# xuangu-fang/Gaussian-Process-Slover-for-High-Freq-PDE

Hardware: AMD Instinct MI355X
Metric: log-joint iters/sec + fp64 Cholesky GFLOP/s, 2D Poisson 256^2, 1-8 GPU (higher is better)
Workload: dtype f64; 1 GPU; C4: 2D Poisson 256x256 Kronecker grid, Matern52_Cos_1d, Q=30, fp64; Q=30, kernel=Matern52_Cos_1d, equation=poisson_2d-sin_sin, parallelism=replicas x1 (one independent problem per GPU)

## Files before the change

gaussian-process-slover-for-high-freq-pde_amd/csrc/gpk_create.cpp:

```cpp
#include <atomic>

#include "gpk_host.h"

static std::atomic<int> g_chain_cap{0};

bool build_classes(const double* x, int n, int P, std::vector<double>& dist, std::vector<int>& cid,
                   std::vector<int>& cbase, int& vmax) {
  cid.assign((size_t)P * P, -1);
  cbase.assign((size_t)n + 1, 0);
  dist.clear();
  vmax = 0;
  double vals[CLS_VMAX];
  for (int k = 0; k < n; ++k) {
    int nv = 0;
    cbase[k] = (int)dist.size();
    for (int j = 0; j + k < n; ++j) {
      const double d = std::fabs(x[j + k] - x[j]);
      int v = 0;
      while (v < nv && !(vals[v] == d)) ++v;
      if (v == nv) {
        if (nv == CLS_VMAX) return false;
        vals[nv++] = d;
        dist.push_back(d);
      }
// ... 137 lines not shown
  A_(h->grad, L.nparams);
  A_(h->m, L.nparams);
  A_(h->v, L.nparams);
  A_(h->Up, nup);
  A_(h->kc, 2);
  A_(h->sc, 1);
  A_(h->count, 1);
  A_(h->loss_slot, 1);
  A_(h->status, 1);
  A_(h->stat_x, 2);
  A_(h->losses, LOSS_CAP);
  A_(h->diag, 8);
  for (int a = 0; a < L.naxes; ++a) {
    const int P = axis_p(L, a);
    A_(h->K[a], (size_t)P * P);
    A_(h->Kb[a], (size_t)P * P);
    A_(h->D[a], (size_t)P * P);
    A_(h->piv[a], spd_big_piv_doubles(P));
    A_(h->ldet[a], P / 32);
    A_(h->Kc[a], (size_t)P * P);
    A_(h->pst[a], 2);
    A_(h->aflag[a], 4 + P / 32);
    if (h->bigspd) A_(h->Zp[a], (size_t)3 * 128 * P);
    if (h->bigspd && h->bigwide && !(p->flags & GPK_FLAG_ONE_SWEEP_UPDATE)) {
      const int T2 = (int)((P + 127) / 128);
      std::vector<unsigned> tab;
      wide_schedule(T2, true, tab);
      A_(h->wsched[a], tab.size());
      if (hipMemcpyAsync(h->wsched[a], tab.data(), tab.size() * sizeof(unsigned), hipMemcpyHostToDevice, h->s) != hipSuccess ||
          hipStreamSynchronize(h->s) != hipSuccess)
        return fail(GPK_EHIP, "upload the update schedule");
    }
    A_(h->cflags[a], (size_t)(P / 32) * (P / 32 + (P1 + P2) / 32) + 2 * (P / 32) + 1);
    A_(h->cgran[a], (size_t)(P / 32) * 2048);
    if (hipMemsetD32Async(h->cgran[a], CHAIN_SENTINEL32, (size_t)(P / 32) * 4096, h->s) != hipSuccess)
      return fail(GPK_EHIP, "initialise the pivot-chain input slots");
    if (h->chain) {
      A_(h->PB2[a], 2 * chain_half(P, h->chain_multi));
      A_(h->cepoch[a], 4);
      if (hipMemsetD32Async(h->PB2[a], CHAIN_SENTINEL32, 4 * chain_half(P, h->chain_multi), h->s) != hipSuccess)
        return fail(GPK_EHIP, "initialise the panel slots");
    }
    if (h->chain_aug) {
      A_(h->PD[a], (size_t)P * P);
      A_(h->PBa[a], (size_t)P * (P1 + P2));
    }
    h->nldet[a] = P / 32;
  }
  if (L.dim == 2) {
    A_(h->A, nup); A_(h->Bt, nup); A_(h->S, nup); A_(h->R, nup);
    A_(h->T1, nup); A_(h->T2, nup); A_(h->X1, nup); A_(h->X2, nup);
    A_(h->W1, nup); A_(h->W2, nup); A_(h->Y1, nup); A_(h->Y2, nup);
    for (int a = 0; a < 2; ++a) {
      const int P = axis_p(L, a);
      A_(h->GK[a], (size_t)P * P);
      A_(h->GD[a], (size_t)P * P);
    }
    h->nquad = h->negap = (P1 / 16) * (P2 / 16);
  } else {
    A_(h->alpha, P1); A_(h->R, P1); A_(h->tvec, P1); A_(h->beta, P1); A_(h->rvec, P1);
    if (p->uoff) A_(h->uoff, P1);
    h->nquad = h->negap = gemv_blocks(P1);
  }
  if (shard) {
    const size_t npg = (size_t)L.naxes * 3 * QMAX;
    A_(h->sred, 2 + npg + (size_t)h->negap + (size_t)h->nquad);
    h->stat_x = h->sred;
    h->pg = h->sred + 2;
// ... 259 lines not shown
```

gaussian-process-slover-for-high-freq-pde_amd/csrc/gpk_internal.h:

```cpp
#pragma once
#include <vector>
#include <hip/hip_runtime.h>
#include <stdint.h>

namespace gpk {

constexpr int QMAX = 64;
constexpr int PADM = 32;
constexpr int NB = 32;
constexpr double SQRT5 = 2.23606797749978969641;
constexpr double TWO_PI = 6.28318530717958647692;

enum Kind { SE_COS = 0, MATERN52_COS = 1, SE = 2, MATERN52 = 3 };

__host__ __device__ inline bool kind_matern(int k) { return k == MATERN52_COS || k == MATERN52; }
__host__ __device__ inline bool kind_cos(int k) { return k == SE_COS || k == MATERN52_COS; }
inline int pad_up(int n) { return (n + PADM - 1) / PADM * PADM; }

struct AxisConst {
  double w[QMAX];
  double a[QMAX];
  double om[QMAX];
  double oml[QMAX];
};
// ... 138 lines not shown
  double* Y;
  int p;
  int n;
  double* piv;
  double* ldet;
  double* pst;
  int* status;
  unsigned int* flag;
  int wide;
  int no_quarters;
  int qfirst;
  double* Z;
  const unsigned* sched;
};
int wide_sched_stride(int T2);
void wide_schedule(int T2, bool paired, std::vector<unsigned>& tab);
hipError_t launch_spd_inverse(SpdArgs* args, int nmat, double** final_out, hipStream_t s,
                              bool pivot0_done = false);
hipError_t launch_spd_stage(SpdArgs* args, int nmat, int stage, hipStream_t s);

constexpr int CHAIN_MAX_BLOCKS = 512;
struct ChainArgs {
  double* X; double* PB; double* piv; double* ldet; double* pst; int* status;
  unsigned int* flags;
  int p, n;
  const int* cid; const double* kval; const double* dval; const double* x; double jitter;
  double* Kc; double* D;
  int tu, td;
  const double* Bu; int ldbu, bu_t;
  double* Ou; int ldou, ou_t;
  double* Od; int ldod;
  double* PBa; int ldpba;
  double* gran;
  double* PB2; unsigned int* epoch;
};
__host__ __device__ inline size_t multi_half(int p) { return (size_t)p * p + (size_t)32 * p; }
__host__ __device__ inline size_t chain_half(int p, bool multi) { return multi ? multi_half(p) : (size_t)32 * p; }
constexpr unsigned long long CHAIN_SENTINEL = 0x7ff4dead7ff4deadull;
constexpr unsigned int CHAIN_SENTINEL32 = 0x7ff4deadu;
int spd_chain_blocks(const int* p, int nmat, bool aug);
int spd_chain_capacity(int deriv, bool gather);
__host__ __device__ inline int chain_role(int m, int x, int T, int TC) {
  const int nt = T * TC, nc = 2 * (T - 1);
  auto crit = [TC](int i) { return (i & 1) ? ((i >> 1) + 1) * (TC + 1) : (i >> 1) * (TC + 1) + 1; };
  int r;
  if (m == 0) {
    if (x == nt) return nt;
    if (x >= nt - nc) return crit(x - (nt - nc));
    r = x;
  } else {
    if (x == 0) return nt;
    if (x <= nc) return crit(x - 1);
    r = x - 1 - nc;
  }
  int tile = r;
  for (int i = 0; i < nc; ++i)
    if (crit(i) <= tile) ++tile;
  return tile;
}
int spd_chain_multi_blocks(const int* p, int nmat);
int spd_chain_multi_capacity(int deriv, bool gather);
hipError_t launch_spd_chain_multi(const ChainArgs* a, int nmat, int deriv, hipStream_t s,
                                  const PrepArgs* prep = nullptr, int q = 0);
hipError_t launch_spd_chain(const ChainArgs* a, int nmat, int deriv, hipStream_t s,
                            const PrepArgs* prep = nullptr, int q = 0);

// ... 103 lines not shown
```

gaussian-process-slover-for-high-freq-pde_amd/csrc/gpk_step.cpp:

```cpp
#include <sched.h>

#include <atomic>

#include "gpk_host.h"

namespace {
const char* kStageNames1D[] = {"prep", "assemble", "spd_inverse", "gemv_alpha", "gemv_alpha_res",
                               "gemv_alpha_fix", "gemv_resid", "gemv_DtR", "gemv_beta",
                               "gemv_beta_res", "gemv_beta_fix", "pgrad_tail"};
const char* kStageNames2D[] = {"prep", "assemble", "spd_inverse", "gemm_A", "gemm_A_res",
                               "gemm_A_fix", "gemm_B", "gemm_B_res", "gemm_B_fix", "gemm_C",
                               "gemm_D", "gemm_D_res", "gemm_D_fix", "gemm_E", "pgrad_tail"};
}

static void mark(gpk_handle* h, int stage) {
  if (h->profiling) (void)hipEventRecord(h->ev[stage + 1], h->s);
}

PrepArgs make_prep(gpk_handle* h, int apply) {
  const Layout& L = h->L;
  PrepArgs P{};
  P.params = h->params;
  P.off_kp[0] = L.off_kp[0];
  P.off_kp[1] = L.off_kp[1];
// ... 19 lines not shown
  return !h->shard && h->chain && h->cls[0].ncls > 0 && h->nce_flag &&
         !(h->prob.flags & GPK_FLAG_NO_CLASS_PIPE);
}

void fill_spd(gpk_handle* h, SpdArgs* sa) {
  const Layout& L = h->L;
  for (int a = 0; a < L.naxes; ++a) {
    sa[a] = SpdArgs{};
    sa[a].X = h->K[a];
    sa[a].Y = h->Kb[a];
    sa[a].p = axis_p(L, a);
    sa[a].n = axis_n(L, a);
    sa[a].piv = h->piv[a];
    sa[a].ldet = h->ldet[a];
    sa[a].status = h->status;
    sa[a].pst = h->pst[a];
    sa[a].flag = h->aflag[a];
    sa[a].wide = h->bigwide ? 1 : 0;
    sa[a].no_quarters = (h->prob.flags & GPK_FLAG_NO_QUARTER_TILES) ? 1 : 0;
    sa[a].qfirst = (h->prob.flags & GPK_FLAG_NO_QUARTER_FIRST) ? 0 : 1;
    sa[a].Z = h->Zp[a];
    sa[a].sched = h->wsched[a];
  }
}

hipError_t launch_chain(gpk_handle* h, bool gather, double** fin, bool aug, const PrepArgs* prep) {
  const Layout& L = h->L;
  ChainArgs ca[2] = {};
  for (int a = 0; a < L.naxes; ++a) {
    ChainArgs& c = ca[a];
    c.X = h->K[a]; c.PB = h->Kb[a]; c.piv = h->piv[a]; c.ldet = h->ldet[a]; c.pst = h->pst[a];
    c.status = h->status; c.flags = h->cflags[a]; c.gran = h->cgran[a];
    c.PB2 = h->PB2[a]; c.epoch = h->cepoch[a];
    c.p = axis_p(L, a);
    c.n = axis_n(L, a);
    if (gather) {
      c.cid = h->cls[a].cid; c.kval = h->cls[a].kval; c.dval = h->cls[a].dval;
      c.x = axis_x(h, a); c.jitter = h->prob.jitter; c.Kc = h->Kc[a];
    }
    c.D = h->D[a];
    if (gather && h->cls_gemv) c.Kc = c.D = nullptr;
    if (h->chain_aug && aug) {
      c.tu = axis_p(L, 1 - a) / 32; c.td = c.p / 32;
      c.Bu = h->Up; c.ldbu = L.p2; c.bu_t = a;
      c.Ou = a ? h->Bt : h->A; c.ldou = L.p2; c.ou_t = a;
      c.Od = h->PD[a]; c.ldod = c.p;
      c.PBa = h->PBa[a]; c.ldpba = L.p1 + L.p2;
    }
    fin[a] = h->K[a];
  }
  if (h->chain_multi) return launch_spd_chain_multi(ca, L.naxes, step_deriv(h), h->s, prep, L.q);
  return launch_spd_chain(ca, L.naxes, step_deriv(h), h->s, prep, L.q);
}

hipError_t launch_inverse(gpk_handle* h, SpdArgs* sa, double** fin, bool pivot0_done) {
  if (h->bigspd) return launch_spd_inverse_big(sa, h->L.naxes, fin, h->s);
  if (h->chain) return launch_chain(h, false, fin, false);
  return launch_spd_inverse(sa, h->L.naxes, fin, h->s, pivot0_done);
}

void fill_assemble(const gpk_handle* h, AssembleArgs* aa) {
  for (int a = 0; a < h->L.naxes; ++a) {
    aa[a] = AssembleArgs{};
    aa[a].x = axis_x(h, a);
    aa[a].n = axis_n(h->L, a);
    aa[a].p = axis_p(h->L, a);
// ... 474 lines not shown
  h->fold_report = nullptr;
  if (rc != GPK_OK) return rc;
  if (pending_begin) return fail(GPK_EINVAL, "internal: the batch begin was not folded into a step");
  if (pending_report || h->shard) return check_launch(launch_step_report(*r, h->s), "step_report");
  return GPK_OK;
}

static int capture_whole(gpk_handle* h, hipGraphExec_t* slot, bool fast, int reps) {
  if (*slot) return GPK_OK;
  const StepBegin b = make_begin(h, fast);
  const StepReport rep = make_report(h, fast, reps);
  return capture_graph(h->s, slot, [&] {
    int rc = begin_batch(h, &b);
    if (rc == GPK_OK) rc = enqueue_steps(h, 1, !fast, reps, &rep);
    return end_batch(h, &rep, rc);
  });
}

static int capture_call(gpk_handle* h, bool fast) {
  return capture_whole(h, &h->g_call[fast ? 0 : 1], fast, 1);
}

static int capture_calln(gpk_handle* h, int reps) {
  const int rc = capture_whole(h, &h->g_calln[reps], true, reps);
  if (rc != GPK_OK) h->g_calln.erase(reps);
  return rc;
}

int reset_handoffs(gpk_handle* h) {
  const Layout& L = h->L;
  for (int a = 0; a < L.naxes; ++a) {
    const size_t P = axis_p(L, a), T = P / 32;
    const size_t nflags = T * (T + (L.p1 + L.p2) / 32) + 2 * T + 1;
    HIPCHK(hipMemsetD32Async(h->cgran[a], CHAIN_SENTINEL32, T * 4096, h->s));
    if (h->PB2[a]) HIPCHK(hipMemsetD32Async(h->PB2[a], CHAIN_SENTINEL32, 4 * chain_half((int)P, h->chain_multi), h->s));
    if (h->cepoch[a]) HIPCHK(hipMemsetAsync(h->cepoch[a], 0, 4 * sizeof(unsigned int), h->s));
    HIPCHK(hipMemsetAsync(h->cflags[a], 0, nflags * sizeof(unsigned int), h->s));
    HIPCHK(hipMemsetAsync(h->aflag[a], 0, (4 + P / 32) * sizeof(unsigned int), h->s));
  }
  HIPCHK(hipMemsetAsync(h->nce_flag, 0, sizeof(unsigned int), h->s));
  HIPCHK(hipStreamSynchronize(h->s));
  return GPK_OK;
}

int status_error(int st, int* status, hipStream_t s, gpk_handle* h, bool undo_batch, bool handoffs) {
  const bool timeout = handoffs && (st & 2);
  HIPCHK(hipMemsetAsync(status, 0, sizeof(int), s));
  if (timeout) TRY(reset_handoffs(h));
  if (undo_batch) {
    TRY(restore_snapshot(h));
    HIPCHK(hipStreamSynchronize(s));
  }
  const std::string msg =
      timeout ? "SPD inverse: a pivot-chain hand-off timed out (device status 2)"
              : "covariance factor is not positive definite (non-positive pivot in SPD inverse)";
  return fail(GPK_ENOTPD, undo_batch ? msg + "; the batch was undone" : msg);
}

int read_status(gpk_handle* h) {
  int st = 0;
  HIPCHK(hipMemcpyAsync(&st, h->status, sizeof(int), hipMemcpyDeviceToHost, h->s));
  HIPCHK(hipStreamSynchronize(h->s));
  return st ? status_error(st, h->status, h->s, h, false, true) : GPK_OK;
}

constexpr double FAST_GRAPH_MARGIN = 2.0;
static int read_report(gpk_handle* h, bool fast, bool* violated);
// ... 228 lines not shown
```

gaussian-process-slover-for-high-freq-pde_amd/csrc/gpk_trace.h:

```cpp
#pragma once
#include <hip/hip_runtime.h>
#include <stdint.h>

namespace gpk {

constexpr int TRACE_SLOTS = 256;
enum TraceSlot {
  SLOT_CLASS_EVAL = 0, SLOT_GATHER = 1, SLOT_PIVOT0_WAIT = 2, SLOT_PIVOT0 = 3,
  SLOT_SWEEP = 4,
  SLOT_SWEEP_PIVOT = 20,
  SLOT_PREFETCH_MISS = 36,
  SLOT_PG_GARR = 37,
  SLOT_PG_ULAST = 38,
  SLOT_CLASS_SUM = 40, SLOT_PGRAD = 41, SLOT_PG_CONTRACT = 42, SLOT_PG_GROUP = 43,
  SLOT_PG_TOP = 44, SLOT_PG_UPLANE = 45, SLOT_PG_FINAL = 46,
  SLOT_PG_START = 47, SLOT_PG_STAGED = 48, SLOT_CSUM_START = 49, SLOT_CEVAL_START = 50,
  SLOT_GATHER_START = 51, SLOT_CSUM_LOADED = 52, SLOT_CHAIN_END = 53, SLOT_CHAIN_M1 = 54,
  SLOT_LAST_FLAG = 58, SLOT_LAST_LDS = 59, SLOT_LAST_MMA = 60, SLOT_LAST_OUT = 61, SLOT_LAST_AUG = 62,
  SLOT_GEMM = 64,
  SLOT_MC_PANEL = 128,
  SLOT_MC_PIV = 144,
  SLOT_MC_LDS = 160,
  SLOT_MC_V = 176,
  SLOT_MC_PUB = 192,
  SLOT_MC_DONE = 208,
  SLOT_MC_PROD = 224,
  SLOT_MCP_IN = 64, SLOT_MCP_OUT = 240,
  SLOT_MCP_WHO_IN = 80, SLOT_MCP_WHO_OUT = 96, SLOT_MCP_MPOS = 112,
  SLOT_BIG_START = 240, SLOT_BIG_PIVTILE = 241, SLOT_BIG_PIVOT = 242, SLOT_BIG_PANEL_WAIT = 243,
  SLOT_BIG_PANEL = 244, SLOT_BIG_ROUND0 = 245, SLOT_BIG_ROUND1 = 246, SLOT_BIG_QUARTER = 247,
  SLOT_BIG_R0START = 248,
};
constexpr int BIG_PROBE_SWEEP = 8;

#ifdef GPK_TRACE
#define GPK_TRACE_TU(tu)                                                                  \
  namespace {                                                                             \
  __device__ unsigned long long trace_lo[TRACE_SLOTS], trace_hi[TRACE_SLOTS];             \
  }                                                                                       \
  void trace_fetch_##tu(uint64_t* lo, uint64_t* hi) {                                     \
    (void)hipMemcpyFromSymbol(lo, HIP_SYMBOL(trace_lo), sizeof(trace_lo));                \
    (void)hipMemcpyFromSymbol(hi, HIP_SYMBOL(trace_hi), sizeof(trace_hi));                \
  }                                                                                       \
  void trace_reset_##tu() {                                                               \
    unsigned long long lo[TRACE_SLOTS], hi[TRACE_SLOTS];                                  \
    for (int i = 0; i < TRACE_SLOTS; ++i) lo[i] = ~0ull, hi[i] = 0ull;                    \
// ... 36 lines not shown
```

gaussian-process-slover-for-high-freq-pde_amd/csrc/spdinv.hip:

```cpp
#include <algorithm>

#include "gpk_internal.h"
#include "spd_pivot.h"
#include "gpk_trace.h"
#include "prep_dev.h"

namespace gpk {

GPK_WAIT_LIMIT_SETTER(wait_limit_spdinv)

GPK_TRACE_TU(spdinv)

typedef double d4 __attribute__((ext_vector_type(4)));

constexpr int SA = 34;
constexpr int SB = 48;
struct SpdBatch {
  double* X[2];
  double* Y[2];
  int p[2];
  int T[2];
  double* piv[2];
  double* ldet[2];
  double* pst[2];
// ... 115 lines not shown
    __syncthreads();
    if (t == 0) {
      double mx = 0.0;
      for (int j = 0; j < 32; ++j) mx = fmax(mx, pv[j]);
      atomicMax(reinterpret_cast<unsigned long long*>(b.pst[m] + 1),
                (unsigned long long)__double_as_longlong(mx));
    }
    if (trb) TR_HI(SLOT_SWEEP + k);
    return;
  }
  if (!nextpiv) {
    if (trb) TR_HI(SLOT_SWEEP + k);
    return;
  }
  __syncthreads();
  if (trb) TR_LO(SLOT_SWEEP_PIVOT + k);
  const double ls = pivot_chol_inv_1w(sP, sM, pv, t, b.status[m]);
  double* piv = b.piv[m] + (size_t)(k + 1) * 1024;
  for (int e = t; e < 1024; e += 256) piv[e] = sM[(e >> 5) * SP + (e & 31)];
  if (t == 0) b.ldet[m][k + 1] = ls;
  if (trb) TR_HI(SLOT_SWEEP_PIVOT + k);
  if (trb) TR_HI(SLOT_SWEEP + k);
}

struct ChainFactor {
  double* X;
  double* PB;
  double* piv;
  double* ldet;
  double* pst;
  int* status;
  unsigned int* flags;
  double* gran;
  double* PB2;
  unsigned int* epoch;
  int piv_off;
  int p, n, T;
  const int* cid; const double* kval; const double* dval; const double* x; double jitter;
  double* Kc; double* D;
  int tu, td;
  const double* Bu; int ldbu, bu_t;
  double* Ou; int ldou, ou_t;
  double* Od; int ldod;
  double* PBa; int ldpba;
};
struct ChainBatch {
  ChainFactor f[2];
  int nmat;
  PrepArgs prep;
  int q;
  int mpos;
};

__device__ __forceinline__ void st_sc1(double* p, double v) {
  __hip_atomic_store(p, v, __ATOMIC_RELAXED, __HIP_MEMORY_SCOPE_AGENT);
}
__device__ __forceinline__ double ld_sc1(const double* p) {
  return __hip_atomic_load(const_cast<double*>(p), __ATOMIC_RELAXED, __HIP_MEMORY_SCOPE_AGENT);
}
__device__ __forceinline__ void wait_flag(unsigned int* f, int* status) {
  (void)spin_until_ge<1>(f, 1u, status);
}
__device__ __forceinline__ void signal_flag(unsigned int* f) {
  asm volatile("s_waitcnt vmcnt(0)" ::: "memory");
  __syncthreads();
  if (threadIdx.x == 0) __hip_atomic_store(f, 1u, __ATOMIC_RELAXED, __HIP_MEMORY_SCOPE_AGENT);
}

__device__ __forceinline__ double* gran_at(const ChainFactor& F, int slot, int which, int e) {
  return F.gran + (size_t)(2 * slot + which) * 1024 + e;
}
__device__ __forceinline__ bool gran_ok(double v) {
  return __double_as_longlong(v) != (long long)CHAIN_SENTINEL;
}

template <bool ONEWAVE>
__device__ __forceinline__ void chain_master(const ChainFactor& F, int T, d4 acc, double* sXJ,
                                             double* sP, double* sM, double* pv, bool trm,
                                             bool early_flag, double* lw = nullptr) {
  const int t = threadIdx.x, lane = t & 63, wv = t >> 6;
  const int wr = wv >> 1, wc = wv & 1;
  const int tx = t & 31, ty = t >> 5;
  unsigned int* piv_rdy = F.flags + F.piv_off;
  __shared__ int s_pflag;
  __builtin_amdgcn_s_setprio(3);
  auto ex = [&](int r) { return (ty + 8 * r) * 32 + tx; };
  auto ed = [&](int r) { return (16 * wr + (lane >> 4) + 4 * r) * 32 + 16 * wc + (lane & 15); };
  double gx[4], gd[4];
  auto issue = [&](int k) {
#pragma unroll
    for (int r = 0; r < 4; ++r) {
      gx[r] = ld_sc1(gran_at(F, k, 0, ex(r)));
      gd[r] = ld_sc1(gran_at(F, k, 1, ed(r)));
    }
  };
  struct PivotPrefetch {
    __device__ constexpr bool waves() const { return true; }
    decltype(issue)* f;
    int k, T;
    __device__ void early() {}
    __device__ void pre() {}
    __device__ void post() {
      if (k + 1 < T) (*f)(k);
    }
  };
  auto factor = [&](int kp) {
    if (trm && kp > 0 && kp < 17) TR_HI(SLOT_SWEEP + kp - 1);
    store_quad(sP, SP, wr, wc, lane, acc);
    __syncthreads();
    if (trm && kp > 0 && kp < 17) TR_LO(SLOT_SWEEP_PIVOT + kp - 1);
    if (trm && kp == 0) TR_LO(SLOT_PIVOT0);
    PivotPrefetch hook{&issue, kp, T};
// ... 57 lines not shown
  }
}

template <int DERIV, bool GATHER>
__global__ __launch_bounds__(256, 2) void chain_kernel(ChainBatch b) {
  const int m = blockIdx.y;
  if (m == b.nmat) {
    if (blockIdx.x == 0) publish_prep(b.prep, b.q);
    copy_snapshot(b.prep, blockIdx.x, gridDim.x);
    return;
  }
  const ChainFactor& F = b.f[m];
  const int T = F.T, p = F.p;
  const int TC = T + F.tu + F.td;
  if ((int)blockIdx.x > T * TC) return;
  const int tile = chain_role(m, (int)blockIdx.x, T, TC);
  const bool master = tile == T * TC;
  const int I = master ? 0 : tile / TC, J = master ? 0 : tile % TC;
  const bool aug = J >= T;
  const int ja = J - T;
  const int t = threadIdx.x, lane = t & 63, wv = t >> 6;
  const int wr = wv >> 1, wc = wv & 1;
  const int tx = t & 31, ty = t >> 5;
  unsigned int* panel_rdy = F.flags;
  unsigned int* piv_rdy = F.flags + T * TC;
  unsigned int* done = F.flags + T * TC + 2 * T;
  auto panel_ptr = [&](int k, int row, int col) -> double* {
    return J < T ? F.PB + (size_t)(k * 32 + row) * p + J * 32 + col
                 : F.PBa + (size_t)(k * 32 + row) * F.ldpba + ja * 32 + col;
  };
  __shared__ double sL[32 * SA];
  __shared__ double sXI[32 * SB], sXJ[32 * SB];
  __shared__ double sP[32 * SP], sM[32 * SP], pv[32];
  __shared__ unsigned int s_last;
  const unsigned ep = F.PB2 ? __hip_atomic_load(F.epoch, __ATOMIC_RELAXED, __HIP_MEMORY_SCOPE_AGENT) : 0u;
  double* PLc = F.PB2 ? F.PB2 + (size_t)(ep & 1u) * chain_half(p, false) : nullptr;

  d4 acc;
#pragma unroll
  for (int r = 0; r < 4; ++r) {
    const int i = I * 32 + 16 * wr + (lane >> 4) + 4 * r, j = J * 32 + 16 * wc + (lane & 15);
    const size_t o = (size_t)i * p + j;
    if (aug) {
      const int jl = ja * 32 + 16 * wc + (lane & 15);
      if (ja < F.tu) {
        acc[r] = F.bu_t ? F.Bu[(size_t)(jl) * F.ldbu + i] : F.Bu[(size_t)i * F.ldbu + jl];
      } else {
        const int jd = jl - 32 * F.tu;
        const size_t od = (size_t)jd * p + i;
        if (GATHER) {
          const int u = F.cid[od];
          double dv = u >= 0 ? F.dval[u] : 0.0;
          if (DERIV == 1 && u >= 0 && !(F.x[jd] - F.x[i] >= 0.0)) dv = -dv;
          acc[r] = dv;
        } else {
          acc[r] = F.D[od];
        }
      }
      continue;
    }
    if (GATHER) {
      const int u = F.cid[o];
      double kv, dv;
      if (u >= 0) {
        kv = F.kval[u];
        if (i == j) kv += F.jitter;
        dv = F.dval[u];
        if (DERIV == 1 && !(F.x[i] - F.x[j] >= 0.0)) dv = -dv;
      } else {
        kv = (i == j) ? 1.0 : 0.0;
        dv = 0.0;
      }
      if (!master) {
        if (F.Kc) F.Kc[o] = kv;
        if (DERIV && F.D) F.D[o] = dv;
      }
      acc[r] = kv;
    } else {
      acc[r] = F.X[o];
    }
  }
  auto publish_tile = [&](void) {
#pragma unroll
    for (int r = 0; r < 4; ++r) st_sc1(panel_ptr(I, 16 * wr + (lane >> 4) + 4 * r, 16 * wc + (lane & 15)), acc[r]);
    signal_flag(panel_rdy + I * TC + J);
  };
  auto chain_inputs = [&](int kk) {
    const int which = (I == kk && J == kk + 1) ? 0 : (I == J && I == kk + 1) ? 1 : -1;
    if (which < 0 || kk + 1 >= T) return;
#pragma unroll
    for (int r = 0; r < 4; ++r)
      st_sc1(gran_at(F, kk, which, (16 * wr + (lane >> 4) + 4 * r) * 32 + 16 * wc + (lane & 15)), acc[r]);
  };
  const bool trm = t == 0 && m == 0;
  if (master) {
    chain_master<true>(F, T, acc, sXJ, sP, sM, pv, trm, false, PLc);
  } else {
    if (trm && tile == 0) TR_LO(SLOT_GATHER);
    chain_inputs(0);
    if (I == 0 && J != 0) publish_tile();
    if (PLc) {
      double* PLo = F.PB2 + (size_t)((ep & 1u) ^ 1u) * chain_half(p, false);
      const int share = (T * 1024 + T * TC - 1) / (T * TC);
      const int e1 = min(T * 1024, (tile + 1) * share);
      for (int e = tile * share + t; e < e1; e += 256) PLo[e] = __longlong_as_double((long long)CHAIN_SENTINEL);
    }
  }

  for (int k = 0; k < T && !master; ++k) {
    const bool needI = I != k, needJ = J != k && J != I;
    if (I == k + 1 || (I == k + 2 && J == k + 2)) __builtin_amdgcn_s_setprio(2);
    else __builtin_amdgcn_s_setprio(0);
    if (t == 0) {
      if (needI) wait_flag(panel_rdy + k * TC + I, F.status);
      if (needJ) wait_flag(panel_rdy + k * TC + J, F.status);
    }
    __syncthreads();
    double xi[4], xj[4];
#pragma unroll
    for (int r = 0; r < 4; ++r) {
      const int row = ty + 8 * r;
      xi[r] = needI ? ld_sc1(F.PB + (size_t)(k * 32 + row) * p + I * 32 + tx) : 0.0;
      xj[r] = needJ ? ld_sc1(panel_ptr(k, row, tx)) : 0.0;
    }
    const bool trl = t == 0 && m == 0 && k == T - 1 && I == T - 1 && J == T - 1;
    double lv[4];
    if (PLc) {
      const double* Lw = PLc + (size_t)k * 1024;
      if (t == 0) {
// ... 521 lines not shown

int spd_chain_multi_blocks(const int* p, int nmat) {
  int w = 0;
  for (int m = 0; m < nmat; ++m) w = std::max(w, multi_workgroups(p[m] / 32));
  return w * nmat;
}

int spd_chain_blocks(const int* p, int nmat, bool aug) {
  int blocks = 0, cols = 0;
  for (int m = 0; m < nmat; ++m) cols += p[m] / 32;
  for (int m = 0; m < nmat; ++m) blocks += (p[m] / 32) * (p[m] / 32 + (aug ? cols : 0)) + 1;
  return blocks;
}

hipError_t launch_spd_chain(const ChainArgs* a, int nmat, int deriv, hipStream_t s,
                            const PrepArgs* prep, int q) {
  ChainBatch b{};
  b.nmat = nmat;
  if (prep) {
    b.prep = *prep;
    b.q = q;
  }
  int Tmax = 0;
  bool gather = a[0].cid != nullptr;
  for (int m = 0; m < nmat; ++m) {
    ChainFactor& f = b.f[m];
    f.X = a[m].X; f.PB = a[m].PB; f.piv = a[m].piv; f.ldet = a[m].ldet; f.pst = a[m].pst;
    f.status = a[m].status; f.flags = a[m].flags; f.p = a[m].p; f.n = a[m].n; f.T = a[m].p / 32;
    f.cid = a[m].cid; f.kval = a[m].kval; f.dval = a[m].dval; f.x = a[m].x; f.jitter = a[m].jitter;
    f.Kc = a[m].Kc; f.D = a[m].D;
    f.tu = a[m].tu; f.td = a[m].td; f.Bu = a[m].Bu; f.ldbu = a[m].ldbu; f.bu_t = a[m].bu_t;
    f.Ou = a[m].Ou; f.ldou = a[m].ldou; f.ou_t = a[m].ou_t; f.Od = a[m].Od; f.ldod = a[m].ldod;
    f.PBa = a[m].PBa; f.ldpba = a[m].ldpba;
    f.gran = a[m].gran; f.piv_off = f.T * (f.T + f.tu + f.td);
    f.PB2 = a[m].PB2; f.epoch = a[m].epoch;
    if ((a[m].cid != nullptr) != gather || !f.gran || !f.PB2 != !f.epoch) return hipErrorInvalidValue;
    Tmax = std::max(Tmax, f.T * (f.T + f.tu + f.td) + 1);
  }
  dim3 grid(Tmax, nmat + (prep ? 1 : 0));
  if (!gather)
    hipLaunchKernelGGL((chain_kernel<0, false>), grid, dim3(256), 0, s, b);
  else if (deriv == 1)
    hipLaunchKernelGGL((chain_kernel<1, true>), grid, dim3(256), 0, s, b);
  else
    hipLaunchKernelGGL((chain_kernel<2, true>), grid, dim3(256), 0, s, b);
  return hipGetLastError();
}

hipError_t launch_spd_chain_multi(const ChainArgs* a, int nmat, int deriv, hipStream_t s,
                                  const PrepArgs* prep, int q) {
  ChainBatch b{};
  b.nmat = nmat;
  if (prep) {
    b.prep = *prep;
    b.q = q;
  }
  int wmax = 0;
  const bool gather = a[0].cid != nullptr;
  for (int m = 0; m < nmat; ++m) {
    ChainFactor& f = b.f[m];
    f.X = a[m].X; f.PB = a[m].PB; f.piv = a[m].piv; f.ldet = a[m].ldet; f.pst = a[m].pst;
    f.status = a[m].status; f.flags = a[m].flags; f.p = a[m].p; f.n = a[m].n; f.T = a[m].p / 32;
    f.cid = a[m].cid; f.kval = a[m].kval; f.dval = a[m].dval; f.x = a[m].x; f.jitter = a[m].jitter;
    f.Kc = a[m].Kc; f.D = a[m].D;
    f.gran = a[m].gran; f.piv_off = f.T * f.T; f.PB2 = a[m].PB2; f.epoch = a[m].epoch;
    if ((a[m].cid != nullptr) != gather || a[m].tu || a[m].td || !f.gran || !f.PB2 || !f.epoch)
      return hipErrorInvalidValue;
// ... 59 lines not shown
```

gaussian-process-slover-for-high-freq-pde_amd/gpk/_lib.py:

```python
import ctypes
import os

import numpy as np

_HERE = os.path.dirname(os.path.abspath(__file__))
LIB_PATH = os.environ.get("GPK_LIB_PATH") or os.path.join(_HERE, "_lib", "libgpk.so")

GPK_OK, GPK_EINVAL, GPK_ENOTPD, GPK_EHIP, GPK_ERCCL, GPK_ENOMEM, GPK_ENODEV = range(7)
GPK_FLAG_FORCE_BIG_GEMM = 1
GPK_FLAG_FORCE_BIG_SPD = 2
GPK_FLAG_FORCE_SMALL_SPD = 4
GPK_FLAG_FORCE_HUGE_GEMM = 8
GPK_FLAG_NO_FAST_GRAPH = 16
GPK_FLAG_FAST_FIRST = 32
GPK_FLAG_NO_DCLASS = 64
GPK_FLAG_NO_CHAIN = 128
GPK_FLAG_NO_CHAIN_AUG = 256
GPK_FLAG_FORCE_WIDE_SPD = 512
GPK_FLAG_FORCE_NARROW_SPD = 1024
GPK_FLAG_SPLIT_FACTORS = 2048
GPK_FLAG_FORCE_CHAIN_MULTI = 4096
GPK_FLAG_REFINE_ALL = 8192
GPK_FLAG_NO_REFINE = 16384
GPK_FLAG_MATRIX_GEMV = 32768
GPK_FLAG_NO_QUARTER_TILES = 65536
GPK_FLAG_DD_CONTRACTION = 131072
GPK_FLAG_NO_DD_CONTRACTION = 262144
GPK_FLAG_ONE_SWEEP_UPDATE = 524288
GPK_FLAG_NO_QUARTER_FIRST = 1048576
GPK_FLAG_REFINE_FWD1_ONLY = 2097152
GPK_FLAG_NO_CLASS_BINS = 4194304
GPK_FLAG_NO_CLASS_PIPE = 8388608
GPK_INV_SWEEP, GPK_INV_CHAIN, GPK_INV_CHAIN_AUG, GPK_INV_BIG, GPK_INV_BIG_WIDE, GPK_INV_CHAIN_MULTI = range(6)
INV_PATH_NAMES = {0: "sweep", 1: "chain", 2: "chain_aug", 3: "big", 4: "big_wide", 5: "chain_multi"}
KIND_IDS = {"SE_Cos_1d": 0, "Matern52_Cos_1d": 1, "SE_1d": 2, "Matern52_1d": 3}
EQ_IDS = {"poisson": 0, "allencahn": 1, "advection": 2}

_dp = ctypes.POINTER(ctypes.c_double)
_ip = ctypes.POINTER(ctypes.c_int32)


class GPKError(RuntimeError):
    def __init__(self, code, msg):
        super().__init__(f"libgpk error {code}: {msg}")
        self.code = code


class NotPositiveDefinite(GPKError):
    pass


class gpk_problem(ctypes.Structure):
    _fields_ = [
        ("dim", ctypes.c_int32), ("eq", ctypes.c_int32), ("kind", ctypes.c_int32),
        ("n1", ctypes.c_int32), ("n2", ctypes.c_int32), ("q", ctypes.c_int32),
        ("x1", _dp), ("x2", _dp), ("src", _dp), ("bvals", _dp), ("bidx", _ip),
        ("nb", ctypes.c_int32),
        ("jitter", ctypes.c_double), ("llk_weight", ctypes.c_double),
        ("logdet", ctypes.c_double), ("beta", ctypes.c_double),
        ("lr", ctypes.c_double), ("b1", ctypes.c_double), ("b2", ctypes.c_double),
        ("eps", ctypes.c_double),
        ("device", ctypes.c_int32), ("flags", ctypes.c_int32),
        ("uoff", _dp),
    ]

# ... 135 lines not shown
```

include/gpk.h:

```cpp
#ifndef GPK_H_
#define GPK_H_

#include <stdint.h>

#ifdef __cplusplus
extern "C" {
#endif

#define GPK_ABI_VERSION 2

enum {
  GPK_OK = 0,
  GPK_EINVAL = 1,
  GPK_ENOTPD = 2,
  GPK_EHIP = 3,
  GPK_ERCCL = 4,
  GPK_ENOMEM = 5,
  GPK_ENODEV = 6
};

enum { GPK_SE_COS = 0, GPK_MATERN52_COS = 1, GPK_SE = 2, GPK_MATERN52 = 3 };

enum { GPK_POISSON = 0, GPK_ALLENCAHN = 1, GPK_ADVECTION = 2 };

// ... 13 lines not shown
  double llk_weight;
  double logdet;
  double beta;
  double lr, b1, b2, eps;
  int32_t device;
  int32_t flags;
  const double* uoff;
} gpk_problem;

#define GPK_FLAG_FORCE_BIG_GEMM 1
#define GPK_FLAG_FORCE_BIG_SPD 2
#define GPK_FLAG_FORCE_SMALL_SPD 4
#define GPK_FLAG_FORCE_HUGE_GEMM 8
#define GPK_FLAG_NO_FAST_GRAPH 16
#define GPK_FLAG_FAST_FIRST 32
#define GPK_FLAG_NO_DCLASS 64
#define GPK_FLAG_NO_CHAIN 128
#define GPK_FLAG_NO_CHAIN_AUG 256
#define GPK_FLAG_FORCE_WIDE_SPD 512
#define GPK_FLAG_FORCE_NARROW_SPD 1024
#define GPK_FLAG_SPLIT_FACTORS 2048
#define GPK_FLAG_FORCE_CHAIN_MULTI 4096
#define GPK_FLAG_REFINE_ALL 8192
#define GPK_FLAG_NO_REFINE 16384
#define GPK_FLAG_MATRIX_GEMV 32768
#define GPK_FLAG_NO_QUARTER_TILES 65536
#define GPK_FLAG_DD_CONTRACTION 131072
#define GPK_FLAG_NO_DD_CONTRACTION 262144
#define GPK_FLAG_ONE_SWEEP_UPDATE 524288
#define GPK_FLAG_NO_QUARTER_FIRST 1048576
#define GPK_FLAG_REFINE_FWD1_ONLY 2097152
#define GPK_FLAG_NO_CLASS_BINS 4194304
#define GPK_FLAG_NO_CLASS_PIPE 8388608

typedef struct gpk_handle gpk_handle;

int gpk_abi_version(void);
const char* gpk_last_error(void);
int gpk_device_count(int32_t* n);

int gpk_kernel_matrices(int32_t kind, int32_t deriv, const double* x1, int32_t n1,
                        const double* x2, int32_t n2, const double* logw, const double* logls,
                        const double* freq, int32_t q, double jitter, double* K_out,
                        double* D_out);

int gpk_kernel_pairs(int32_t kind, int32_t deriv, const double* x1, const double* x2, int64_t n,
                     const double* logw, const double* logls, const double* freq, int32_t q,
                     double* out);

int gpk_create(const gpk_problem* prob, double freq_scale, gpk_handle** out);
int gpk_destroy(gpk_handle* h);

enum { GPK_INV_SWEEP = 0, GPK_INV_CHAIN = 1, GPK_INV_CHAIN_AUG = 2, GPK_INV_BIG = 3, GPK_INV_BIG_WIDE = 4,
       GPK_INV_CHAIN_MULTI = 5 };
int gpk_inverse_path(const gpk_handle* h, int32_t* path);
int gpk_set_chain_capacity(int32_t workgroups);
int gpk_set_spd_big_workgroups(int32_t workgroups);
int gpk_set_wait_limit(int32_t polls);
int gpk_set_wait_limit_chunk(int32_t polls, int32_t chunk);

int gpk_graph_mode(const gpk_handle* h, int32_t* fast, int64_t* rollbacks);

int gpk_distance_classes(const double* x, int32_t n, int32_t* ncls, int32_t* vmax);
int gpk_class_count(const gpk_handle* h, int32_t axis, int32_t* ncls);
int gpk_class_sum_path(const gpk_handle* h, int32_t* epilogue);
int gpk_class_pipe(const gpk_handle* h, int32_t* on);
// ... 81 lines not shown
```

Measured before the change: 10150 iters/s.

## Add lookahead to chained block Cholesky master to overlap next-pivot update

Adds a lookahead path to the chain master: while one wave factors the current 32x32 pivot, the other waves pull the next panel's inputs from a three-slot granule buffer and apply the trailing update for the following diagonal block with f64 MFMA. Worker tiles now publish inputs two steps ahead, so the sequential pivot chain is meant to stop waiting on the serial update between pivots. The granule buffer grows from two to three slots per step, which adds memory, memset cost and shared memory use. A new flag disables the path.

```diff
diff --git a/gaussian-process-slover-for-high-freq-pde_amd/csrc/gpk_create.cpp b/gaussian-process-slover-for-high-freq-pde_amd/csrc/gpk_create.cpp
--- a/gaussian-process-slover-for-high-freq-pde_amd/csrc/gpk_create.cpp
+++ b/gaussian-process-slover-for-high-freq-pde_amd/csrc/gpk_create.cpp
@@ -193,8 +193,8 @@
         return fail(GPK_EHIP, "upload the update schedule");
     }
     A_(h->cflags[a], (size_t)(P / 32) * (P / 32 + (P1 + P2) / 32) + 2 * (P / 32) + 1);
-    A_(h->cgran[a], (size_t)(P / 32) * 2048);
-    if (hipMemsetD32Async(h->cgran[a], CHAIN_SENTINEL32, (size_t)(P / 32) * 4096, h->s) != hipSuccess)
+    A_(h->cgran[a], (size_t)(P / 32) * 3072);
+    if (hipMemsetD32Async(h->cgran[a], CHAIN_SENTINEL32, (size_t)(P / 32) * 6144, h->s) != hipSuccess)
       return fail(GPK_EHIP, "initialise the pivot-chain input slots");
     if (h->chain) {
       A_(h->PB2[a], 2 * chain_half(P, h->chain_multi));
diff --git a/gaussian-process-slover-for-high-freq-pde_amd/csrc/gpk_internal.h b/gaussian-process-slover-for-high-freq-pde_amd/csrc/gpk_internal.h
--- a/gaussian-process-slover-for-high-freq-pde_amd/csrc/gpk_internal.h
+++ b/gaussian-process-slover-for-high-freq-pde_amd/csrc/gpk_internal.h
@@ -194,6 +194,7 @@
   double* Od; int ldod;
   double* PBa; int ldpba;
   double* gran;
+  int lookahead;
   double* PB2; unsigned int* epoch;
 };
 __host__ __device__ inline size_t multi_half(int p) { return (size_t)p * p + (size_t)32 * p; }
diff --git a/gaussian-process-slover-for-high-freq-pde_amd/csrc/gpk_step.cpp b/gaussian-process-slover-for-high-freq-pde_amd/csrc/gpk_step.cpp
--- a/gaussian-process-slover-for-high-freq-pde_amd/csrc/gpk_step.cpp
+++ b/gaussian-process-slover-for-high-freq-pde_amd/csrc/gpk_step.cpp
@@ -75,6 +75,7 @@
     c.X = h->K[a]; c.PB = h->Kb[a]; c.piv = h->piv[a]; c.ldet = h->ldet[a]; c.pst = h->pst[a];
     c.status = h->status; c.flags = h->cflags[a]; c.gran = h->cgran[a];
     c.PB2 = h->PB2[a]; c.epoch = h->cepoch[a];
+    c.lookahead = (h->prob.flags & GPK_FLAG_NO_CHAIN_LOOKAHEAD) ? 0 : 1;
     c.p = axis_p(L, a);
     c.n = axis_n(L, a);
     if (gather) {
@@ -615,7 +616,7 @@
   for (int a = 0; a < L.naxes; ++a) {
     const size_t P = axis_p(L, a), T = P / 32;
     const size_t nflags = T * (T + (L.p1 + L.p2) / 32) + 2 * T + 1;
-    HIPCHK(hipMemsetD32Async(h->cgran[a], CHAIN_SENTINEL32, T * 4096, h->s));
+    HIPCHK(hipMemsetD32Async(h->cgran[a], CHAIN_SENTINEL32, T * 6144, h->s));
     if (h->PB2[a]) HIPCHK(hipMemsetD32Async(h->PB2[a], CHAIN_SENTINEL32, 4 * chain_half((int)P, h->chain_multi), h->s));
     if (h->cepoch[a]) HIPCHK(hipMemsetAsync(h->cepoch[a], 0, 4 * sizeof(unsigned int), h->s));
     HIPCHK(hipMemsetAsync(h->cflags[a], 0, nflags * sizeof(unsigned int), h->s));
diff --git a/gaussian-process-slover-for-high-freq-pde_amd/csrc/gpk_trace.h b/gaussian-process-slover-for-high-freq-pde_amd/csrc/gpk_trace.h
--- a/gaussian-process-slover-for-high-freq-pde_amd/csrc/gpk_trace.h
+++ b/gaussian-process-slover-for-high-freq-pde_amd/csrc/gpk_trace.h
@@ -12,6 +12,7 @@
   SLOT_PREFETCH_MISS = 36,
   SLOT_PG_GARR = 37,
   SLOT_PG_ULAST = 38,
+  SLOT_LOOKAHEAD_LATE = 39,
   SLOT_CLASS_SUM = 40, SLOT_PGRAD = 41, SLOT_PG_CONTRACT = 42, SLOT_PG_GROUP = 43,
   SLOT_PG_TOP = 44, SLOT_PG_UPLANE = 45, SLOT_PG_FINAL = 46,
   SLOT_PG_START = 47, SLOT_PG_STAGED = 48, SLOT_CSUM_START = 49, SLOT_CEVAL_START = 50,
diff --git a/gaussian-process-slover-for-high-freq-pde_amd/csrc/spdinv.hip b/gaussian-process-slover-for-high-freq-pde_amd/csrc/spdinv.hip
--- a/gaussian-process-slover-for-high-freq-pde_amd/csrc/spdinv.hip
+++ b/gaussian-process-slover-for-high-freq-pde_amd/csrc/spdinv.hip
@@ -171,6 +171,7 @@
   int* status;
   unsigned int* flags;
   double* gran;
+  int la;
   double* PB2;
   unsigned int* epoch;
   int piv_off;
@@ -209,14 +210,194 @@
 __device__ __forceinline__ double* gran_at(const ChainFactor& F, int slot, int which, int e) {
   return F.gran + (size_t)(2 * slot + which) * 1024 + e;
 }
+__device__ __forceinline__ double* gran3_at(const ChainFactor& F, int slot, int which, int e) {
+  return F.gran + (size_t)(3 * slot + which) * 1024 + e;
+}
 __device__ __forceinline__ bool gran_ok(double v) {
   return __double_as_longlong(v) != (long long)CHAIN_SENTINEL;
 }
 
-template <bool ONEWAVE>
+__device__ __forceinline__ d4 mma_r(const double (&a)[8], const double (&b)[8], d4 acc) {
+#pragma unroll
+  for (int kk = 0; kk < 8; ++kk) acc = __builtin_amdgcn_mfma_f64_16x16x4f64(a[kk], b[kk], acc, 0, 0, 0);
+  return acc;
+}
+__device__ __forceinline__ d4 mma_lr(const double* a, int sai, int sak, const double (&b)[8], int wr,
+                                     int lane, d4 acc) {
+  const int li = lane & 15, lk = lane >> 4;
+#pragma unroll
+  for (int kk = 0; kk < 8; ++kk)
+    acc = __builtin_amdgcn_mfma_f64_16x16x4f64(a[(16 * wr + li) * sai + (4 * kk + lk) * sak], b[kk], acc, 0, 0, 0);
+  return acc;
+}
+
+struct NoTileSource {
+  __device__ double operator()(int, int) const { return 0.0; }
+};
+
+template <class KF>
+__device__ __forceinline__ void chain_master_la(const ChainFactor& F, int T, d4 acc, double* sX,
+                                                double* sX2, double* sP, double* sM, double* sM2,
+                                                double* sD, double* pv, bool trm, bool trla,
+                                                double* lw, KF kf) {
+  const int t = threadIdx.x, lane = t & 63, wv = t >> 6;
+  const int wr = wv >> 1, wc = wv & 1;
+  int li = lane & 15, lk = lane >> 4;
+  int wq = __builtin_amdgcn_readfirstlane(wv), c = 0, nw = 0;
+  auto fresh_lane = [&]() {
+    int l = lane, w = __builtin_amdgcn_readfirstlane(wv);
+    asm volatile("" : "+v"(l), "+s"(w));
+    li = l & 15;
+    lk = l >> 4;
+    wq = w;
+    c = wq == 2 ? 1 : 0;
+    nw = wq == 3 ? 24 : 20;
+  };
+  unsigned int* piv_rdy = F.flags + F.piv_off;
+  __builtin_amdgcn_s_setprio(3);
+  const double snan = __longlong_as_double((long long)CHAIN_SENTINEL);
+  auto woff = [&](int i) -> int {
+    if (i < 8) return 128 * i + 16 * c;
+    if (i < 16) return wq == 3 ? 16 + 128 * (i - 8) : 1024 + 512 * ((i - 8) >> 2) + 128 * (i & 3) + 16 * c;
+    if (i < 20) return 2048 + 128 * (i & 3) + (wq == 3 ? 16 : 528 * c);
+    return 2048 + 512 + 128 * (i & 3);
+  };
+  auto lookahead = [&](int h) {
+    double* sV1 = (h & 1) ? sX2 : sX;
+    double* sQn = (h & 1) ? sX : sX2;
+    const double* Lh = (h & 1) ? sM2 : sM;
+    fresh_lane();
+    const double* g = gran3_at(F, h, 0, 32 * lk + li);
+    double w[24];
+    for (unsigned spins = 0;; ++spins) {
+      bool ok = true;
+#pragma unroll
+      for (int i = 0; i < 24; ++i) {
+        w[i] = i < nw ? ld_sc1(g + woff(i)) : 0.0;
+        ok = ok && gran_ok(w[i]);
+      }
+#ifdef GPK_TRACE
+      const bool late = spins == 0 && __any(!ok);
+      if (trla && late) { TR_LO(SLOT_LOOKAHEAD_LATE); TR_HI(SLOT_LOOKAHEAD_LATE); }
+#endif
+      if (ok || spin_give_up(spins, F.status)) break;
+      __builtin_amdgcn_s_sleep(1);
+    }
+    const d4 zero = {0.0, 0.0, 0.0, 0.0};
+    double pa[8], va[8];
+#pragma unroll
+    for (int i = 0; i < 8; ++i) pa[i] = w[i];
+    const d4 v0 = mma_lr(Lh, SP, 1, pa, 0, lane, zero), v1 = mma_lr(Lh, SP, 1, pa, 1, lane, zero);
+#pragma unroll
+    for (int i = 0; i < 4; ++i) { va[i] = v0[i]; va[4 + i] = v1[i]; }
+    if (wq != 3) {
+      d4 q0 = {w[8], w[9], w[10], w[11]}, q1 = {w[12], w[13], w[14], w[15]};
+      d4 d2 = {w[16], w[17], w[18], w[19]};
+      q0 = q0 - mma_lr(sV1, 1, SB, va, 0, lane, zero);
+      q1 = q1 - mma_lr(sV1, 1, SB, va, 1, lane, zero);
+      d2 = d2 - mma_r(va, va, zero);
+#pragma unroll
+      for (int r = 0; r < 4; ++r) {
+        sQn[(lk + 4 * r) * SB + 16 * c + li] = q0[r];
+        sQn[(16 + lk + 4 * r) * SB + 16 * c + li] = q1[r];
+        sD[(16 * c + lk + 4 * r) * SP + 16 * c + li] = d2[r];
+      }
+    } else {
+      double pb[8], vb[8];
+#pragma unroll
+      for (int i = 0; i < 8; ++i) pb[i] = w[8 + i];
+      const d4 u0 = mma_lr(Lh, SP, 1, pb, 0, lane, zero), u1 = mma_lr(Lh, SP, 1, pb, 1, lane, zero);
+#pragma unroll
+      for (int i = 0; i < 4; ++i) { vb[i] = u0[i]; vb[4 + i] = u1[i]; }
+      d4 d01 = {w[16], w[17], w[18], w[19]}, d10 = {w[20], w[21], w[22], w[23]};
+      d01 = d01 - mma_r(va, vb, zero);
+      d10 = d10 - mma_r(vb, va, zero);
+#pragma unroll
+      for (int r = 0; r < 4; ++r) {
+        sD[(lk + 4 * r) * SP + 16 + li] = d01[r];
+        sD[(16 + lk + 4 * r) * SP + li] = d10[r];
+      }
+    }
+  };
+  auto rearm = [&](int h) {
+    fresh_lane();
+    double* g = gran3_at(F, h, 0, 32 * lk + li);
+#pragma unroll
+    for (int i = 0; i < 24; ++i)
+      if (i < nw && !(wq == 3 && i < 16)) st_sc1(g + woff(i), snan);
+  };
+  auto factor = [&](int kp) {
+    if (trm && kp > 0 && kp < 17) TR_HI(SLOT_SWEEP + kp - 1);
+    store_quad(sP, SP, wr, wc, lane, acc);
+    __syncthreads();
+    if (trm && kp > 0 && kp < 17) TR_LO(SLOT_SWEEP_PIVOT + kp - 1);
+    if (trm && kp == 0) TR_LO(SLOT_PIVOT0);
+    double* Mk = (kp & 1) ? sM2 : sM;
+    if (wv > 0) {
+      if (kp >= 2) rearm(kp - 2);
+      if (kp == 0 && T > 1) {
+#pragma unroll
+        for (int it = 0; it < 11; ++it) {
+          const int e = t - 64 + 192 * it;
+          if (e >= 2048) continue;
+          const int row = (e >> 5) & 31, col = e & 31;
+          if (e < 1024) sX[row * SB + col] = kf(row, 32 + col);
+          else sD[row * SP + col] = kf(32 + row, 32 + col);
+        }
+      } else if (kp > 0 && kp + 1 < T) {
+        lookahead(kp - 1);
+      }
+    }
+    const double ls = pivot_chol_inv_1w<double*, NoPivotHook>(sP, Mk, pv, t, F.status);
+    double* ldst = (lw ? lw : F.piv) + (size_t)kp * 1024;
+    for (int e = t; e < 1024; e += 256) st_sc1(ldst + e, Mk[(e >> 5) * SP + (e & 31)]);
+    if (t == 0) F.ldet[kp] = ls;
+    if (kp + 1 == T && !lw) signal_flag(piv_rdy + kp);
+    if (trm && kp > 0 && kp < 17) TR_HI(SLOT_SWEEP_PIVOT + kp - 1);
+    if (trm && kp == 0) TR_HI(SLOT_PIVOT0);
+  };
+  if (t == 0) {
+    st_sc1(F.pst, acc[0]);
+    __hip_atomic_store(reinterpret_cast<unsigned long long*>(F.pst + 1), 0ull, __ATOMIC_RELAXED,
+                       __HIP_MEMORY_SCOPE_AGENT);
+  }
+  if (lw) asm volatile("s_waitcnt vmcnt(0)" ::: "memory");
+  factor(0);
+  for (int h = 0; h + 1 < T; ++h) {
+    if (trm && h < 16) TR_LO(SLOT_SWEEP + h);
+    double* sXh = (h & 1) ? sX2 : sX;
+    const double* Lh = (h & 1) ? sM2 : sM;
+#pragma unroll
+    for (int r = 0; r < 4; ++r) acc[r] = sD[(16 * wr + lk + 4 * r) * SP + 16 * wc + li];
+    d4 vj = {0.0, 0.0, 0.0, 0.0};
+    vj = mma_t(Lh, SP, 1, sXh, SB, 1, wr, wc, lane, vj);
+    if (!lw) asm volatile("s_waitcnt vmcnt(0)" ::: "memory");
+    __syncthreads();
+    if (t == 0 && !lw) __hip_atomic_store(piv_rdy + h, 1u, __ATOMIC_RELAXED, __HIP_MEMORY_SCOPE_AGENT);
+    store_quad(sXh, SB, wr, wc, lane, vj);
+    __syncthreads();
+    d4 prod = {0.0, 0.0, 0.0, 0.0};
+    prod = mma_t(sXh, 1, SB, sXh, SB, 1, wr, wc, lane, prod);
+    acc = acc - prod;
+    factor(h + 1);
+  }
+}
+
+struct ChainWindow {
+  double *sX2, *sM2, *sD;
+  bool trla;
+};
+template <bool ONEWAVE, bool LOOKAHEAD = false, class KF = NoTileSource>
 __device__ __forceinline__ void chain_master(const ChainFactor& F, int T, d4 acc, double* sXJ,
                                              double* sP, double* sM, double* pv, bool trm,
-                                             bool early_flag, double* lw = nullptr) {
+                                             bool early_flag, double* lw = nullptr,
+                                             ChainWindow win = ChainWindow(), KF kf = KF()) {
+  if constexpr (LOOKAHEAD) {
+    if (F.la) {
+      chain_master_la(F, T, acc, sXJ, win.sX2, sP, sM, win.sM2, win.sD, pv, trm, win.trla, lw, kf);
+      return;
+    }
+  }
   const int t = threadIdx.x, lane = t & 63, wv = t >> 6;
   const int wr = wv >> 1, wc = wv & 1;
   const int tx = t & 31, ty = t >> 5;
@@ -340,6 +521,7 @@
   __shared__ double sL[32 * SA];
   __shared__ double sXI[32 * SB], sXJ[32 * SB];
   __shared__ double sP[32 * SP], sM[32 * SP], pv[32];
+  __shared__ double sD[32 * SP];
   __shared__ unsigned int s_last;
   const unsigned ep = F.PB2 ? __hip_atomic_load(F.epoch, __ATOMIC_RELAXED, __HIP_MEMORY_SCOPE_AGENT) : 0u;
   double* PLc = F.PB2 ? F.PB2 + (size_t)(ep & 1u) * chain_half(p, false) : nullptr;
@@ -394,15 +576,34 @@
     signal_flag(panel_rdy + I * TC + J);
   };
   auto chain_inputs = [&](int kk) {
-    const int which = (I == kk && J == kk + 1) ? 0 : (I == J && I == kk + 1) ? 1 : -1;
-    if (which < 0 || kk + 1 >= T) return;
+    int which;
+    if (F.la) {
+      which = (J != kk + 2 || kk + 2 >= T) ? -1 : I - kk;
+      if (which < 0 || which > 2) return;
+    } else {
+      which = (I == kk && J == kk + 1) ? 0 : (I == J && I == kk + 1) ? 1 : -1;
+      if (which < 0 || kk + 1 >= T) return;
+    }
+    double* slot = F.la ? gran3_at(F, kk, which, 0) : gran_at(F, kk, which, 0);
 #pragma unroll
     for (int r = 0; r < 4; ++r)
-      st_sc1(gran_at(F, kk, which, (16 * wr + (lane >> 4) + 4 * r) * 32 + 16 * wc + (lane & 15)), acc[r]);
+      st_sc1(slot + (16 * wr + (lane >> 4) + 4 * r) * 32 + 16 * wc + (lane & 15), acc[r]);
+  };
+  auto k_at = [&](int i, int j) -> double {
+    const size_t o = (size_t)i * p + j;
+    if (GATHER) {
+      const int u = F.cid[o];
+      if (u < 0) return (i == j) ? 1.0 : 0.0;
+      double kv = F.kval[u];
+      if (i == j) kv += F.jitter;
+      return kv;
+    }
+    return F.X[o];
   };
   const bool trm = t == 0 && m == 0;
   if (master) {
-    chain_master<true>(F, T, acc, sXJ, sP, sM, pv, trm, false, PLc);
+    const ChainWindow win{sXI, sL, sD, t == 64 && m == 0};
+    chain_master<true, true>(F, T, acc, sXJ, sP, sM, pv, trm, false, PLc, win, k_at);
   } else {
     if (trm && tile == 0) TR_LO(SLOT_GATHER);
     chain_inputs(0);
@@ -990,7 +1191,7 @@
     f.tu = a[m].tu; f.td = a[m].td; f.Bu = a[m].Bu; f.ldbu = a[m].ldbu; f.bu_t = a[m].bu_t;
     f.Ou = a[m].Ou; f.ldou = a[m].ldou; f.ou_t = a[m].ou_t; f.Od = a[m].Od; f.ldod = a[m].ldod;
     f.PBa = a[m].PBa; f.ldpba = a[m].ldpba;
-    f.gran = a[m].gran; f.piv_off = f.T * (f.T + f.tu + f.td);
+    f.gran = a[m].gran; f.piv_off = f.T * (f.T + f.tu + f.td); f.la = a[m].lookahead;
     f.PB2 = a[m].PB2; f.epoch = a[m].epoch;
     if ((a[m].cid != nullptr) != gather || !f.gran || !f.PB2 != !f.epoch) return hipErrorInvalidValue;
     Tmax = std::max(Tmax, f.T * (f.T + f.tu + f.td) + 1);
diff --git a/gaussian-process-slover-for-high-freq-pde_amd/gpk/_lib.py b/gaussian-process-slover-for-high-freq-pde_amd/gpk/_lib.py
--- a/gaussian-process-slover-for-high-freq-pde_amd/gpk/_lib.py
+++ b/gaussian-process-slover-for-high-freq-pde_amd/gpk/_lib.py
@@ -31,6 +31,7 @@
 GPK_FLAG_REFINE_FWD1_ONLY = 2097152
 GPK_FLAG_NO_CLASS_BINS = 4194304
 GPK_FLAG_NO_CLASS_PIPE = 8388608
+GPK_FLAG_NO_CHAIN_LOOKAHEAD = 16777216
 GPK_INV_SWEEP, GPK_INV_CHAIN, GPK_INV_CHAIN_AUG, GPK_INV_BIG, GPK_INV_BIG_WIDE, GPK_INV_CHAIN_MULTI = range(6)
 INV_PATH_NAMES = {0: "sweep", 1: "chain", 2: "chain_aug", 3: "big", 4: "big_wide", 5: "chain_multi"}
 KIND_IDS = {"SE_Cos_1d": 0, "Matern52_Cos_1d": 1, "SE_1d": 2, "Matern52_1d": 3}
diff --git a/include/gpk.h b/include/gpk.h
--- a/include/gpk.h
+++ b/include/gpk.h
@@ -69,6 +69,7 @@
 #define GPK_FLAG_REFINE_FWD1_ONLY 2097152
 #define GPK_FLAG_NO_CLASS_BINS 4194304
 #define GPK_FLAG_NO_CLASS_PIPE 8388608
+#define GPK_FLAG_NO_CHAIN_LOOKAHEAD 16777216
 
 typedef struct gpk_handle gpk_handle;
 
```

Result: faster. 10310 iters/s (median of 6 runs) (+1.5%).
